# intuitive-robots/beso

Hardware: AMD Instinct MI355X
Metric: denoising-steps/sec (score-GPT fwd) at kitchen obs-dim (higher is better)
Workload: dtype bf16; 1 GPU; BASELINE.json configs[1]: Franka kitchen score-GPT fwd (GCDenoiser.forward), batch=4096 synthetic obs/goal per GPU, 1 NFE per step; obs_dim=30, act_dim=9, window=4, goal_seq_len=2, embed_dim=360, n_layers=6, n_heads=6, batch_per_gpu=4096, parallelism=batch-sharded x1, no collective in the loop, weights=seeded N(0,0.02) recipe (no trained checkpoints shipped)

## Files before the change

### beso_amd/csrc/fused.hip

```cpp
#include <stdlib.h>
#include "fused.h"

#ifndef BESO_OPERAND_F16
#define BESO_OPERAND_F16 0
#endif
#if BESO_OPERAND_F16
#define fused_packed_bytes fused_packed_bytes_f16
#define fused_pack fused_pack_f16
#define fused_level fused_level_f16
#define fused_layer_edges fused_layer_edges_f16
#define fused_layers fused_layers_f16
#define fused_can_loop fused_can_loop_f16
#endif

namespace beso {

typedef __attribute__((ext_vector_type(2))) float f32x2;
typedef __attribute__((ext_vector_type(2))) unsigned int u32x2;

template <int B, int E, typename F>
__device__ __forceinline__ void static_for(F&& f) {
    if constexpr (B < E) {
        f(std::integral_constant<int, B>{});
        static_for<B + 1, E>(f);
// ... 99 lines not shown

constexpr bool kt16(int KS) { return KS == 12 || KS == 8; }

bool shape_has_kernel(const FusedDims& d) {
    if (kt16(d.KS) && d.D > 32 * (d.KS - 1) + 16) return false;
    return (d.RPW == 3 && d.KS == 12) || (d.RPW == 2 && d.KS == 8) || (d.RPW == 4 && d.KS == 16);
}

#if BESO_OPERAND_F16
typedef __attribute__((ext_vector_type(2))) _Float16 f16x2;
typedef __attribute__((ext_vector_type(4))) _Float16 f16x4;
typedef __attribute__((ext_vector_type(8))) _Float16 f16x8;
__device__ __forceinline__ uint16_t f2op(float v) { return __builtin_bit_cast(uint16_t, (_Float16)v); }
__device__ __forceinline__ float op2f(uint16_t h) { return (float)__builtin_bit_cast(_Float16, h); }
#else
__device__ __forceinline__ uint16_t f2op(float v) { return f2bf(v); }
__device__ __forceinline__ float op2f(uint16_t h) { return bf2f(h); }
#endif
__device__ __forceinline__ uint16_t f2op_part(float v, int part) {
    const uint16_t h = f2op(v);
    return part ? f2op(v - op2f(h)) : h;
}

__global__ void pack_mfma_a_kernel(const float* __restrict__ src, int rows, int cols, const float* __restrict__ colscale,
                                   uint16_t* __restrict__ dst, int rt, int kt, int grp, int part) {
    size_t total = (size_t)rt * kt * 512;
    for (size_t i = (size_t)blockIdx.x * blockDim.x + threadIdx.x; i < total; i += (size_t)gridDim.x * blockDim.x) {
        int j = (int)(i & 7), lane = (int)((i >> 3) & 63);
        size_t tile = i >> 9;
        int rin = (int)(tile % grp);
        int kk = (int)((tile / grp) % kt);
        int R = (int)(tile / ((size_t)grp * kt)) * grp + rin;
        int r = 16 * R + (lane & 15);
        int c = 32 * kk + 16 * (j >> 2) + 4 * (lane >> 4) + (j & 3);
        float v = 0.f;
        if (r < rows && c < cols) {
            v = src[(size_t)r * cols + c];
            if (colscale) v *= colscale[c];
        }
        dst[i] = f2op_part(v, part);
    }
}

__global__ void pack_qkv_kernel(const float* __restrict__ wq, const float* __restrict__ wk, const float* __restrict__ wv,
                                const float* __restrict__ gamma, uint16_t* __restrict__ dst, int D, int H, int hd,
                                int kt, int split) {
    size_t total = (size_t)H * 12 * kt * 512;
    for (size_t i = (size_t)blockIdx.x * blockDim.x + threadIdx.x; i < total; i += (size_t)gridDim.x * blockDim.x) {
        int j = (int)(i & 7), lane = (int)((i >> 3) & 63);
        size_t tile = i >> 9;
        int rt12 = (int)(tile % 12);
        int kk = (int)((tile / 24) % kt);
        int h = 2 * (int)(tile / ((size_t)24 * kt)) + (int)((tile / 12) & 1);
        int R4 = rt12 & 3, part = rt12 >> 2;
        int d = 16 * R4 + (lane & 15);
        int c = 32 * kk + 16 * (j >> 2) + 4 * (lane >> 4) + (j & 3);
        float v = 0.f;
        if (d < hd && c < D) {
            const float* w = part == 0 ? wq : (part == 1 ? wk : wv);
            v = w[(size_t)(h * hd + d) * D + c] * gamma[c];
        }
        dst[i] = f2op_part(v, split);
    }
}

__global__ void fold_qkv_bias_kernel(const float* __restrict__ wq, const float* __restrict__ wk,
                                     const float* __restrict__ wv, const float* __restrict__ bq,
                                     const float* __restrict__ bk, const float* __restrict__ bv,
                                     const float* __restrict__ beta, float* __restrict__ out, int D, int H, int hd) {
    const int i = (blockIdx.x * blockDim.x + threadIdx.x) >> 6, lane = threadIdx.x & 63;
    if (i >= H * 3 * kHDP) return;
    int d = i % kHDP, part = (i / kHDP) % 3, h = i / (3 * kHDP);
    float acc = 0.f;
    if (d < hd) {
        const float* w = part == 0 ? wq : (part == 1 ? wk : wv);
        const float* b = part == 0 ? bq : (part == 1 ? bk : bv);
        const int r = h * hd + d;
        for (int c = lane; c < D; c += 64) acc = fmaf(w[(size_t)r * D + c], beta[c], acc);
        acc = wave_sum(acc) + b[r];
    }
    if (lane == 0) out[i] = acc;
}

__global__ void pack_proj_kernel(const float* __restrict__ wp, uint16_t* __restrict__ dst, int D, int H, int hd, int rt,
                                 int part) {
    const int kt = 2 * H;
    size_t total = (size_t)rt * kt * 512;
    for (size_t i = (size_t)blockIdx.x * blockDim.x + threadIdx.x; i < total; i += (size_t)gridDim.x * blockDim.x) {
        int j = (int)(i & 7), lane = (int)((i >> 3) & 63);
        size_t tile = i >> 9;
        int R = (int)(tile % rt), kk = (int)(tile / rt);
        int o = 16 * R + (lane & 15);
        int h = kk >> 1;
        int d = 32 * (kk & 1) + 16 * (j >> 2) + 4 * (lane >> 4) + (j & 3);
        float v = 0.f;
        if (o < D && d < hd) v = wp[(size_t)o * D + h * hd + d];
        dst[i] = f2op_part(v, part);
    }
}

__global__ void transpose_pad_kernel(const float* __restrict__ src, int rows, int cols, float* __restrict__ dst, int rows_p) {
    int i = blockIdx.x * blockDim.x + threadIdx.x;
    if (i >= cols * rows_p) return;
    int c = i / rows_p, f = i % rows_p;
    dst[i] = f < rows ? src[(size_t)f * cols + c] : 0.f;
}

__global__ void pack_head_kernel(const float* __restrict__ W, const float* __restrict__ b, const float* __restrict__ gamma,
                                 const float* __restrict__ beta, float* __restrict__ Wh, float* __restrict__ bh, int act,
                                 int D, int Dp) {
    int i = blockIdx.x * blockDim.x + threadIdx.x;
    if (i < 16 * Dp) {
        int a = i / Dp, f = i % Dp;
        Wh[i] = (a < act && f < D) ? W[(size_t)a * D + f] * gamma[f] : 0.f;
    }
    if (i < 16) {
        float acc = 0.f;
        if (i < act) {
            acc = b[i];
            for (int f = 0; f < D; ++f) acc = fmaf(W[(size_t)i * D + f], beta[f], acc);
        }
        bh[i] = acc;
    }
}

__global__ void fold_bias_kernel(const float* __restrict__ W, const float* __restrict__ b, const float* __restrict__ beta,
                                 float* __restrict__ out, int rows, int cols, int rows_p) {
    const int r = (blockIdx.x * blockDim.x + threadIdx.x) >> 6, lane = threadIdx.x & 63;
    if (r >= rows_p) return;
    float acc = 0.f;
    if (r < rows) {
        for (int c = lane; c < cols; c += 64) acc = fmaf(W[(size_t)r * cols + c], beta[c], acc);
        acc = wave_sum(acc) + b[r];
    }
// ... 47 lines not shown

__device__ __forceinline__ f32x4 mfma_op16(const uint2& a, const uint2& b, const f32x4& c) {
#if BESO_OPERAND_F16
    return __builtin_amdgcn_mfma_f32_16x16x16f16(__builtin_bit_cast(f16x4, a), __builtin_bit_cast(f16x4, b), c, 0, 0, 0);
#else
    return __builtin_amdgcn_mfma_f32_16x16x16bf16_1k(__builtin_bit_cast(s16x4, a), __builtin_bit_cast(s16x4, b), c, 0, 0, 0);
#endif
}

__device__ __forceinline__ f32x4 mfma_op_half(const u32x4& a, const u32x4& b, const f32x4& c) {
    return mfma_op16(make_uint2(a[0], a[1]), make_uint2(b[0], b[1]), c);
}

#ifndef BESO_TRAIN_FWD_ABL
#define BESO_TRAIN_FWD_ABL 0
#endif
__host__ __device__ constexpr bool zero_pad_instance(int RPW, int NT) { return RPW != 2 && NT >= 5; }
__device__ __forceinline__ void mixed_chain_pad() {
    __builtin_amdgcn_sched_barrier(0);
    asm volatile("s_nop 4\n\ts_nop 4");
    __builtin_amdgcn_sched_barrier(0);
}

#ifndef BESO_FUSED_ABLATE
#define BESO_FUSED_ABLATE 0
#endif
#if BESO_FUSED_ABLATE == 1
#define ABL_KS(x) 0
#define ABL_PTR(base, off) (base)
#else
#define ABL_KS(x) (x)
#define ABL_PTR(base, off) ((base).adv(off))
#endif

struct WPtr {
    __amdgpu_buffer_rsrc_t rs;
    uint32_t so;
    uint32_t lo;
    __device__ __forceinline__ u32x4 at(int frag) const {
        return __builtin_amdgcn_raw_buffer_load_b128(rs, lo, so + (uint32_t)frag * 1024u, 0);
    }
    __device__ __forceinline__ WPtr adv(size_t frags) const { return WPtr{rs, so + (uint32_t)frags * 1024u, lo}; }
};
__device__ __forceinline__ WPtr wptr(const u32x4* uniform_base, int lane) {
    return WPtr{__builtin_amdgcn_make_buffer_rsrc((void*)uniform_base, 0, 0x7fffffff, 0x00020000), 0u, (uint32_t)lane * 16u};
}

template <int R>
__device__ __forceinline__ void prefetch_a(u32x4 (&aE)[R], u32x4 (&aO)[R], WPtr a, int a_ks) {
#pragma unroll
    for (int r = 0; r < R; ++r) { aE[r] = a.at(r); aO[r] = a.at(r + ABL_KS(a_ks)); }
}

template <int R, int NT, bool TAIL16 = false, int NTA = NT>
__device__ __forceinline__ void gemm_phase(f32x4 (&acc)[R][NTA], u32x4 (&aE)[R], u32x4 (&aO)[R],
                                           WPtr a, int a_ks, const u32x4* b, int b_ts,
                                           int b_ks, int ksteps) {
    constexpr int H1 = (NT + 1) / 2;
    u32x4 bf[NT];
#pragma unroll
    for (int t = 0; t < NT; ++t) bf[t] = b[t * b_ts];
    for (int kk = 0; kk < ksteps; kk += 2) {
        __builtin_amdgcn_sched_barrier(0);
#pragma unroll
        for (int t = 0; t < H1; ++t)
#pragma unroll
            for (int r = 0; r < R; ++r) acc[r][t] = mfma_op(aE[r], bf[t], acc[r][t]);
        __builtin_amdgcn_sched_barrier(0);
#pragma unroll
        for (int t = 0; t < H1; ++t) if (!(BESO_ABL_MASK & 32)) bf[t] = b[t * b_ts + (kk + 1) * b_ks];
        __builtin_amdgcn_sched_barrier(0);
#pragma unroll
        for (int t = H1; t < NT; ++t)
#pragma unroll
            for (int r = 0; r < R; ++r) acc[r][t] = mfma_op(aE[r], bf[t], acc[r][t]);
        __builtin_amdgcn_sched_barrier(0);
#pragma unroll
        for (int t = H1; t < NT; ++t) if (!(BESO_ABL_MASK & 32)) bf[t] = b[t * b_ts + (kk + 1) * b_ks];
        if (kk + 2 < ksteps) {
#pragma unroll
            for (int r = 0; r < R; ++r) aE[r] = a.at(r + ABL_KS((kk + 2) * a_ks));
        }
        const bool tail = TAIL16 && kk + 2 >= ksteps;
        __builtin_amdgcn_sched_barrier(0);
        if (tail) {
            mixed_chain_pad();
#pragma unroll
            for (int t = 0; t < NT; ++t)
#pragma unroll
                for (int r = 0; r < R; ++r) acc[r][t] = mfma_op_half(aO[r], bf[t], acc[r][t]);
            break;
        }
#pragma unroll
        for (int t = 0; t < H1; ++t)
#pragma unroll
            for (int r = 0; r < R; ++r) acc[r][t] = mfma_op(aO[r], bf[t], acc[r][t]);
        __builtin_amdgcn_sched_barrier(0);
        if (kk + 2 < ksteps && !(BESO_ABL_MASK & 32)) {
#pragma unroll
            for (int t = 0; t < H1; ++t) bf[t] = b[t * b_ts + (kk + 2) * b_ks];
        }
        __builtin_amdgcn_sched_barrier(0);
#pragma unroll
        for (int t = H1; t < NT; ++t)
#pragma unroll
            for (int r = 0; r < R; ++r) acc[r][t] = mfma_op(aO[r], bf[t], acc[r][t]);
        __builtin_amdgcn_sched_barrier(0);
        if (kk + 2 < ksteps && !(BESO_ABL_MASK & 32)) {
#pragma unroll
            for (int t = H1; t < NT; ++t) bf[t] = b[t * b_ts + (kk + 2) * b_ks];
        }
        if (kk + 3 < ksteps) {
#pragma unroll
            for (int r = 0; r < R; ++r) aO[r] = a.at(r + ABL_KS((kk + 3) * a_ks));
        }
    }
}

template <int R, int PFA>
__device__ __forceinline__ void prefetch_ring(u32x4 (&ar)[PFA][R], WPtr a, int a_ks) {
#pragma unroll
    for (int p = 0; p < PFA; ++p)
#pragma unroll
        for (int r = 0; r < R; ++r) ar[p][r] = a.at(r + ABL_KS(p * a_ks));
}

template <int R, int NT, int PFA, bool TAIL16 = false>
__device__ __forceinline__ void gemm_phase_ring(f32x4 (&acc)[R][NT], u32x4 (&ar)[PFA][R],
                                                WPtr a, int a_ks, const u32x4* b, int b_ts,
                                                int b_ks, int ksteps) {
    static_assert(PFA % 2 == 0, "B fragments alternate between two sets");
    u32x4 bb[2][NT];
#pragma unroll
    for (int t = 0; t < NT; ++t) bb[0][t] = b[t * b_ts];
#pragma unroll
    for (int t = 0; t < NT; ++t) bb[1][t] = b[t * b_ts + b_ks];
    for (int k0 = 0; k0 < ksteps; k0 += PFA) {
#pragma unroll
        for (int p = 0; p < PFA; ++p) {
            const int kk = k0 + p;
            __builtin_amdgcn_sched_barrier(0);
            if (TAIL16 && kk + 1 >= ksteps) {
                mixed_chain_pad();
#pragma unroll
                for (int t = 0; t < NT; ++t)
#pragma unroll
                    for (int r = 0; r < R; ++r) acc[r][t] = mfma_op_half(ar[p][r], bb[p & 1][t], acc[r][t]);
            } else {
#pragma unroll
                for (int t = 0; t < NT; ++t)
#pragma unroll
                    for (int r = 0; r < R; ++r) acc[r][t] = mfma_op(ar[p][r], bb[p & 1][t], acc[r][t]);
            }
            __builtin_amdgcn_sched_barrier(0);
            if (BESO_FUSED_ABLATE != 2 && !(BESO_ABL_MASK & 32) && kk + 2 < ksteps) {
#pragma unroll
                for (int t = 0; t < NT; ++t) bb[p & 1][t] = b[t * b_ts + (kk + 2) * b_ks];
            }
            if (BESO_FUSED_ABLATE != 3 && kk + PFA < ksteps) {
// ... 1075 lines not shown
                            gelu_slot<RC, NT, decltype(SG)::value>(h, gc0, gc1, gq, hb);
                        });
                    });
                    __builtin_amdgcn_sched_barrier(0);
                    if (t == H1 - 1 && kk + 1 < kKC && !(BESO_ABL_MASK & 32)) {
#pragma unroll
                        for (int t2 = 0; t2 < H1; ++t2) bf[t2] = b[t2 * kKC * 64 + (kk + 1) * 64];
                    }
                    if (t == NT - 1) {
                        if (kk + 1 < kKC && !(BESO_ABL_MASK & 32)) {
#pragma unroll
                            for (int t2 = H1; t2 < NT; ++t2) bf[t2] = b[t2 * kKC * 64 + (kk + 1) * 64];
                        }
                        if (kk + 2 < kKC) {
#pragma unroll
                            for (int r = 0; r < RPW; ++r) af2[kk & 1][r] = a2.at(r + ABL_KS((kk + 2) * A2KS));
                        }
                    }
                });
            });
        }
        fc2_prefetch(c);
        stamp(st, 21);
        if (!(BESO_ABL_MASK & 2)) __syncthreads();
        stamp(st, 22);
        constexpr bool kLateG = NT <= 4;
        if (fc1_active) { write_hT(hb); if (!kLateG) keep_g(pc(c), hb); }
        if (c + 1 < n_chunks && next_active) { fc1(c + 1, h, a1r); keep_h(pc(c + 1), h); }
        if (kLateG && fc1_active) keep_g(pc(c), hb);
        stamp(st, 23);
        if (!(BESO_ABL_MASK & 2)) __syncthreads();
        stamp(st, 24);
    }
    {
        const int c = n_chunks - 1;
        const int tiles_here = min(kChunkTiles, HT - pc(c) * kChunkTiles);
        gemm_phase<RPW, NT, false, kNTT>(T.acc, af2[0], af2[1], fc2_a(c), A2KS, hT + lane, kKC * 64, 64, ((tiles_here >> 1) + 1) & ~1);
    }
    stamp(st, 25);
    __syncthreads();
}

__device__ __forceinline__ uint2 v_frag(const uint16_t* qkv, int row0, int dt, int n, int g) {
    typedef s16x4 __attribute__((address_space(3))) * lds_s16x4;
    const uint16_t* p = qkv + ((size_t)2 * kQKVRows + row0 + 4 * g + (n >> 2)) * kQKVRow + 16 * dt + 4 * (n & 3);
    return __builtin_bit_cast(uint2, __builtin_amdgcn_ds_read_tr16_b64_v4i16((lds_s16x4)(p)));
}

template <int KS>
__device__ __forceinline__ void attn_prefetch(u32x4 (&qE)[3], u32x4 (&qO)[3], const u32x4* __restrict__ wqkv, int w, int lane) {
    prefetch_a<3>(qE, qO, wptr(wqkv + (size_t)(3 * w) * 64, lane), 24);
}

template <int RPW, int KS, int HG, int NTP = kNTT, int NTQ = kNTT, class AX = AttnPlain>
__device__ __forceinline__ void attn_phase(Tile<RPW>& T, const u32x4* xnT, unsigned char* u,
                                           const u32x4* __restrict__ wqkv, const float* __restrict__ bqkv,
                                           const u32x4* __restrict__ wproj, int H, int hd, int Tn, int n_samples,
                                           int w, int lane, const SlotTabs* tb, u32x4 (&qE)[3], u32x4 (&qO)[3], Stamps& st,
                                           const AX ax = AX{}) {
    asm volatile("" : "+v"(lane));
    uint16_t* qkv = (uint16_t*)u;
    u32x4* yT = (u32x4*)(u + kQKVBytes);
    const int wa = w & 3, hsel = w >> 2;
    const float scale_log2e = 1.4426950408889634f * __builtin_amdgcn_rsqf((float)hd);
    auto qkv_a = [&](int pair) { return ABL_PTR(wptr(wqkv + (size_t)(3 * w) * 64, lane), (size_t)pair * KS * 24); };
    auto proj_a = [&](int h) { return ABL_PTR(wptr(wproj + (size_t)(w * RPW) * 64, lane), (size_t)(2 * h) * (kWaves * RPW)); };
    int ln = lane;
    auto write_qkv = [&](const f32x4 (&qa)[3][NTQ], int vh) {
        const int n = ln & 15, g = ln >> 4;
        int row[NTQ];
#pragma unroll
        for (int t = 0; t < NTQ; ++t) row[t] = tb->row_of_slot[t * 16 + n];
#pragma unroll
        for (int i = 0; i < 3; ++i) {
            const int rt = 3 * wa + i, part = rt >> 2, d0 = (rt & 3) * 16 + 4 * g;
            uint16_t* dst = qkv + (size_t)part * kQKVRows * kQKVRow + d0;
#pragma unroll
            for (int t = 0; t < NTQ; ++t) {
                uint2 pk;
                pk.x = pack_op2(qa[i][t][0], qa[i][t][1]);
                pk.y = pack_op2(qa[i][t][2], qa[i][t][3]);
                *(uint2*)(dst + (size_t)row[t] * kQKVRow) = pk;
                if constexpr (AX::on) {
                    const int grow = ax.rows.row(t * 16 + n);
                    if (grow >= 0 && d0 < HG * hd && !(BESO_TRAIN_FWD_ABL & 4))
                        *(uint2*)(ax.qkv + (size_t)grow * (3 * ax.D) + part * ax.D + vh * (HG * hd) + d0) = pk;
                }
            }
        }
    };
    const int my_tok = tb->slot_of_row[min(w, n_samples - 1) * Tn + min(lane & 15, Tn - 1)];
    auto drop4 = [&](float (&e)[4], int rh, int n, int g) {
        if constexpr (AX::on) {
            if (ax.p > 0.f) {
                const size_t base = drop_idx_attn((size_t)(ax.s0 + w) * ax.H + rh, Tn, n, 4 * g);
#pragma unroll
                for (int r = 0; r < 4; ++r) e[r] *= drop_scale(ax.seed, ax.site, base + r, ax.p, ax.inv_keep);
            }
        }
    };
    auto keep_y = [&](const auto& yb, int vh, int tok, int g) {
        if constexpr (AX::on) {
            const int grow = ax.rows_y.row(tok);
            if (grow >= 0 && !(BESO_TRAIN_FWD_ABL & 4)) {
                uint16_t* dst = ax.y + (size_t)grow * ax.D + vh * (HG * hd) + 4 * g;
#pragma unroll
                for (int dt = 0; dt < 4; ++dt)
                    if (16 * dt + 4 * g < HG * hd) *(uint2*)(dst + 16 * dt) = make_uint2(yb[dt >> 1][2 * (dt & 1)], yb[dt >> 1][2 * (dt & 1) + 1]);
            }
        }
    };
    auto core = [&](int vh) {
    const int n = ln & 15, g = ln >> 4;
    if constexpr (HG > 1) {
        if (w < n_samples && !(BESO_ABL_MASK & 16)) {
            const uint16_t* qb = qkv + ((size_t)0 * kQKVRows + w * Tn + n) * kQKVRow + 8 * g;
            const uint16_t* kb = qkv + ((size_t)1 * kQKVRows + w * Tn + n) * kQKVRow + 8 * g;
            u32x4 qf[2], kf[2];
#pragma unroll
            for (int kk = 0; kk < 2; ++kk) { qf[kk] = *(const u32x4*)(qb + 32 * kk); kf[kk] = *(const u32x4*)(kb + 32 * kk); }
            uint2 va[4];
#pragma unroll
            for (int dt = 0; dt < 4; ++dt) va[dt] = v_frag(qkv, w * Tn, dt, n, g);
            f32x4 y[4];
#pragma unroll
            for (int dt = 0; dt < 4; ++dt) y[dt] = f32x4{0.f, 0.f, 0.f, 0.f};
#pragma unroll
            for (int h = 0; h < HG; ++h) {
                const int lo_d = h * hd, hi_d = lo_d + hd;
                f32x4 sT = {0.f, 0.f, 0.f, 0.f};
#pragma unroll
// ... 60 lines not shown
        float e[4], m = -INFINITY;
#pragma unroll
        for (int r = 0; r < 4; ++r) {
            e[r] = (4 * g + r <= n) ? sT[r] * scale_log2e : -INFINITY;
            m = fmaxf(m, e[r]);
        }
        m = rows_allreduce<true>(m);
        float sum = 0.f;
#pragma unroll
        for (int r = 0; r < 4; ++r) { e[r] = __builtin_amdgcn_exp2f(e[r] - m); sum += e[r]; }
        sum = rows_allreduce<false>(sum);
        const float inv = __builtin_amdgcn_rcpf(sum);
        if constexpr (AX::on) drop4(e, vh, n, g);
        uint2 pb = make_uint2(pack_op2(e[0], e[1]), pack_op2(e[2], e[3]));
        f32x4 y[4];
#pragma unroll
        for (int dt = 0; dt < 4; ++dt) {
            const uint2 va = v_frag(qkv, w * Tn, dt, n, g);
            const f32x4 z = {0.f, 0.f, 0.f, 0.f};
            y[dt] = mfma_op16(va, pb, z);
        }
        if (n < Tn) {
            const int tok = my_tok;
            u32x4 ybk[AX::on ? 2 : 1];
#pragma unroll
            for (int kk = 0; kk < 2; ++kk) {
                u32x4 yb;
                yb[0] = pack_op2(y[2 * kk][0] * inv, y[2 * kk][1] * inv);
                yb[1] = pack_op2(y[2 * kk][2] * inv, y[2 * kk][3] * inv);
                yb[2] = pack_op2(y[2 * kk + 1][0] * inv, y[2 * kk + 1][1] * inv);
                yb[3] = pack_op2(y[2 * kk + 1][2] * inv, y[2 * kk + 1][3] * inv);
                yT[((size_t)(tok >> 4) * 2 + kk) * 64 + (g << 4) + (tok & 15)] = yb;
                if constexpr (AX::on) ybk[kk] = yb;
            }
            if constexpr (AX::on) keep_y(ybk, vh, tok, g);
        }
    }
    }
    };

    for (int pair = 0; pair < H / 2; ++pair) {
        const int hA = 2 * pair, hB = hA + 1;
        asm volatile("" : "+v"(ln));
        const int g = ln >> 4;
        stamp(st, 10);
        u32x4 aE[RPW], aO[RPW];
        f32x4 qa[3][NTQ];
#pragma unroll
        for (int i = 0; i < 3; ++i) {
            const f32x4 bv = *(const f32x4*)(bqkv + ((hA + hsel) * 12 + 3 * wa + i) * 16 + 4 * g);
#pragma unroll
            for (int t = 0; t < NTQ; ++t) qa[i][t] = bv;
        }
        gemm_phase<3, NTQ, kt16(KS)>(qa, qE, qO, qkv_a(pair), 24, xnT + lane, KS * 64, 64, KS);
        prefetch_a<RPW>(aE, aO, proj_a(hA), kWaves * RPW);
        if (hsel == 0) write_qkv(qa, hA);
        stamp(st, 11);
        __syncthreads();
        stamp(st, 12);
        core(hA);
        stamp(st, 16);
        __syncthreads();
        stamp(st, 17);
        gemm_phase<RPW, NTP, false, kNTT>(T.acc, aE, aO, proj_a(hA), kWaves * RPW, yT + lane, 2 * 64, 64, 2);
        prefetch_a<RPW>(aE, aO, proj_a(hB), kWaves * RPW);
        if (hsel == 1) write_qkv(qa, hB);
        if (pair + 1 < H / 2) prefetch_a<3>(qE, qO, qkv_a(pair + 1), 24);
        stamp(st, 13);
        __syncthreads();
        stamp(st, 14);
        core(hB);
        stamp(st, 15);
        __syncthreads();
        stamp(st, 18);
        gemm_phase<RPW, NTP, false, kNTT>(T.acc, aE, aO, proj_a(hB), kWaves * RPW, yT + lane, 2 * 64, 64, 2);
    }
    __syncthreads();
}

template <int RPW, int KS, int NT>
__device__ __forceinline__ void attn_phase_long(Tile<RPW>& T, const u32x4* xnT, unsigned char* u, const u32x4* __restrict__ wqkv,
                                                const float* __restrict__ bqkv, const u32x4* __restrict__ wproj, int H, int hd,
                                                int Tn, int w, int lane, u32x4 (&qE)[3], u32x4 (&qO)[3], Stamps& st) {
    static_assert(NT == 5, "the wave -> query tile table below");
    asm volatile("" : "+v"(lane));
    constexpr int kRows = 16 * NT, kHead = 3 * kRows * kQKVRow;
    constexpr int kYT = 16 * kQKVRow * 2 / 16;
    uint16_t* qkv = (uint16_t*)u;
    const int wa = w & 3, hsel = w >> 2;
    const float scale_log2e = 1.4426950408889634f * __builtin_amdgcn_rsqf((float)hd);
    auto qkv_a = [&](int pair) { return wptr(wqkv + (size_t)(3 * w) * 64, lane).adv((size_t)pair * KS * 24); };
    auto proj_a = [&](int h) { return wptr(wproj + (size_t)(w * RPW) * 64, lane).adv((size_t)(2 * h) * (kWaves * RPW)); };
    int ln = lane;
    auto core = [&](int head, int qt) {
        const int n = ln & 15, g = ln >> 4;
        uint16_t* hq = qkv + (size_t)head * kHead;
        const uint16_t* qb = hq + ((size_t)16 * qt + n) * kQKVRow + 8 * g;
        const u32x4 q0 = *(const u32x4*)qb, q1 = *(const u32x4*)(qb + 32);
        float e[NT][4];
        float m = -INFINITY;
        const int query = 16 * qt + n;
#pragma unroll
        for (int kt = 0; kt < NT; ++kt) {
            if (kt <= qt) {
                const uint16_t* kb = hq + ((size_t)kRows + 16 * kt + n) * kQKVRow + 8 * g;
                f32x4 sT = {0.f, 0.f, 0.f, 0.f};
                sT = mfma_op(*(const u32x4*)kb, q0, sT);
// ... 12 lines not shown
        for (int kt = 0; kt < NT; ++kt) {
            if (kt <= qt) {
#pragma unroll
                for (int r = 0; r < 4; ++r) { e[kt][r] = __builtin_amdgcn_exp2f(e[kt][r] - m); sum += e[kt][r]; }
            }
        }
        sum = rows_allreduce<false>(sum);
        const float inv = __builtin_amdgcn_rcpf(sum);
        f32x4 y[4];
#pragma unroll
        for (int dt = 0; dt < 4; ++dt) y[dt] = f32x4{0.f, 0.f, 0.f, 0.f};
        typedef s16x4 __attribute__((address_space(3))) * lds_s16x4;
#pragma unroll
        for (int kt = 0; kt < NT; ++kt) {
            if (kt <= qt) {
                const uint2 pb = make_uint2(pack_op2(e[kt][0], e[kt][1]), pack_op2(e[kt][2], e[kt][3]));
#pragma unroll
                for (int dt = 0; dt < 4; ++dt) {
                    const uint16_t* pv = hq + ((size_t)2 * kRows + 16 * kt + 4 * g + (n >> 2)) * kQKVRow + 16 * dt + 4 * (n & 3);
                    const uint2 va = __builtin_bit_cast(uint2, __builtin_amdgcn_ds_read_tr16_b64_v4i16((lds_s16x4)(pv)));
                    y[dt] = mfma_op16(va, pb, y[dt]);
                }
            }
        }
        u32x4* yT = (u32x4*)(hq + (size_t)16 * qt * kQKVRow);
#pragma unroll
        for (int kk = 0; kk < 2; ++kk) {
            u32x4 yb;
            yb[0] = pack_op2(y[2 * kk][0] * inv, y[2 * kk][1] * inv);
            yb[1] = pack_op2(y[2 * kk][2] * inv, y[2 * kk][3] * inv);
            yb[2] = pack_op2(y[2 * kk + 1][0] * inv, y[2 * kk + 1][1] * inv);
            yb[3] = pack_op2(y[2 * kk + 1][2] * inv, y[2 * kk + 1][3] * inv);
            yT[kk * 64 + ln] = yb;
        }
    };
#pragma unroll 1
    for (int pair = 0; pair < H / 2; ++pair) {
        const int hA = 2 * pair, hB = hA + 1;
        asm volatile("" : "+v"(ln));
        const int n = ln & 15, g = ln >> 4;
        stamp(st, 10);
        u32x4 aE[RPW], aO[RPW];
        f32x4 qa[3][NT];
#pragma unroll
        for (int i = 0; i < 3; ++i) {
            const f32x4 bv = *(const f32x4*)(bqkv + ((hA + hsel) * 12 + 3 * wa + i) * 16 + 4 * g);
#pragma unroll
            for (int t = 0; t < NT; ++t) qa[i][t] = bv;
        }
        gemm_phase<3, NT, kt16(KS)>(qa, qE, qO, qkv_a(pair), 24, xnT + lane, KS * 64, 64, KS);
        prefetch_a<RPW>(aE, aO, proj_a(hA), kWaves * RPW);
#pragma unroll
        for (int i = 0; i < 3; ++i) {
            const int rt = 3 * wa + i, part = rt >> 2, d0 = (rt & 3) * 16 + 4 * g;
            uint16_t* dst = qkv + (size_t)hsel * kHead + (size_t)part * kRows * kQKVRow + d0;
#pragma unroll
            for (int t = 0; t < NT; ++t)
                *(uint2*)(dst + (size_t)(16 * t + n) * kQKVRow) =
                    make_uint2(pack_op2(qa[i][t][0], qa[i][t][1]), pack_op2(qa[i][t][2], qa[i][t][3]));
        }
        stamp(st, 11);
        __syncthreads();
        stamp(st, 12);
        if (!(BESO_ABL_MASK & 16)) {
            const int head = w & 1, slot = w >> 1;
            core(head, slot == 0 ? 4 : slot == 1 ? 3 : slot == 2 ? 2 : 1);
            if (slot == 2) core(head, 0);
        }
        if (pair + 1 < H / 2) prefetch_a<3>(qE, qO, qkv_a(pair + 1), 24);
        stamp(st, 16);
        __syncthreads();
        stamp(st, 17);
        gemm_phase<RPW, NT, false, kNTT>(T.acc, aE, aO, proj_a(hA), kWaves * RPW, (const u32x4*)qkv + lane, kYT, 64, 2);
        prefetch_a<RPW>(aE, aO, proj_a(hB), kWaves * RPW);
        gemm_phase<RPW, NT, false, kNTT>(T.acc, aE, aO, proj_a(hB), kWaves * RPW, (const u32x4*)(qkv + kHead) + lane, kYT, 64, 2);
        stamp(st, 13);
        __syncthreads();
        stamp(st, 14);
    }
}

__device__ __forceinline__ float gelu_exact(float v) {
    const float ax = fabsf(v) * 0.70710678118654752440f;
    const float t = __builtin_amdgcn_rcpf(fmaf(0.3275911f, ax, 1.0f));
    float p = fmaf(1.061405429f, t, -1.453152027f);
    p = fmaf(p, t, 1.421413741f);
    p = fmaf(p, t, -0.284496736f);
    p = fmaf(p, t, 0.254829592f);
    p *= t;
    const float ex = __builtin_amdgcn_exp2f(ax * ax * -1.4426950408889634f);
    const float r = fmaf(-p, ex, 1.0f);
    const float hv = 0.5f * v;
    return fmaf(fabsf(hv), r, hv);
}

template <int RPW, int KS, int NW, int NT>
__device__ __forceinline__ void mlp_phase_x3(Tile<RPW>& T, const u32x4* xnT, int xn_lo, u32x4* hT, int h_lo,
                                             const u32x4* __restrict__ w1p, const float* __restrict__ b1f,
                                             const u32x4* __restrict__ w2p, int HT, uint32_t x3_delta, int w, int lane) {
    asm volatile("" : "+v"(lane));
    const int n_chunks = (HT + kChunkTiles - 1) / kChunkTiles;
    constexpr int RC = kChunkTiles / NW, KW = RC / 2;
    constexpr int A2KS = NW * RPW;
#pragma unroll 1
    for (int c = 0; c < n_chunks; ++c) {
        asm volatile("" : "+v"(lane));
        const int g = lane >> 4;
// ... 6 lines not shown
#pragma unroll
            for (int t = 0; t < NT; ++t) h[r][t] = bias;
        }
        if (RC * w < tiles_here)
            gemm_x3<RC, NT, 2, kt16(KS)>(h, wptr(w1p + (size_t)(RC * w) * 64, lane).adv((size_t)c * KS * kChunkTiles), kChunkTiles,
                                      x3_delta, xnT + lane, xn_lo, KS * 64, 64, KS);
        u32x4 hh[KW][NT], hl[KW][NT];
#pragma unroll
        for (int j2 = 0; j2 < KW; ++j2)
#pragma unroll
            for (int t = 0; t < NT; ++t)
#pragma unroll
                for (int q = 0; q < 4; ++q) {
                    const f32x4& hv = h[2 * j2 + (q >> 1)][t];
                    const SplitPair p = split_op2(gelu_exact(hv[2 * (q & 1)]), gelu_exact(hv[2 * (q & 1) + 1]));
                    hh[j2][t][q] = p.hi;
                    hl[j2][t][q] = p.lo;
                }
        if (c > 0) __syncthreads();
#pragma unroll
        for (int j2 = 0; j2 < KW; ++j2)
#pragma unroll
            for (int t = 0; t < NT; ++t) {
                hT[((size_t)t * kKC + KW * w + j2) * 64 + lane] = hh[j2][t];
                hT[((size_t)t * kKC + KW * w + j2) * 64 + lane + h_lo] = hl[j2][t];
            }
        __syncthreads();
        gemm_x3<RPW, NT, 2, false, kNTT>(T.acc, wptr(w2p + (size_t)(w * RPW) * 64, lane).adv((size_t)(c * kKC) * A2KS), A2KS, x3_delta,
                                      hT + lane, h_lo, kKC * 64, 64, ((tiles_here >> 1) + 1) & ~1);
    }
    __syncthreads();
}

template <int RPW, int KS, int HG, int NTP, int NTQ>
__device__ __forceinline__ void attn_phase_x3(Tile<RPW>& T, const u32x4* xnT, int xn_lo, unsigned char* u, int qkv_rows,
                                              int y_off, int y_lo, const u32x4* __restrict__ wqkv,
                                              const float* __restrict__ bqkv, const u32x4* __restrict__ wproj, int H, int hd,
                                              int Tn, int n_samples, uint32_t x3_delta, int w, int lane, const SlotTabs* tb) {
    asm volatile("" : "+v"(lane));
    float* qkv = (float*)u;
    u32x4* yT = (u32x4*)(u + y_off);
    const int wa = w & 3, hsel = w >> 2;
    const float scale_log2e = 1.4426950408889634f * __builtin_amdgcn_rsqf((float)hd);
    auto qkv_a = [&](int pair) { return wptr(wqkv + (size_t)(3 * w) * 64, lane).adv((size_t)pair * KS * 24); };
    auto proj_a = [&](int h) { return wptr(wproj + (size_t)(w * RPW) * 64, lane).adv((size_t)(2 * h) * (kWaves * RPW)); };
    int ln = lane;
    auto write_qkv = [&](const f32x4 (&qa)[3][NTQ]) {
        const int n = ln & 15, g = ln >> 4;
#pragma unroll
        for (int t = 0; t < NTQ; ++t) {
            const int row = tb->row_of_slot[t * 16 + n];
#pragma unroll
            for (int i = 0; i < 3; ++i) {
                const int rt = 3 * wa + i, part = rt >> 2, d0 = (rt & 3) * 16 + 4 * g;
                *(f32x4*)(qkv + ((size_t)part * qkv_rows + row) * kQKVRowF + d0) = qa[i][t];
            }
        }
    };
    auto core = [&]() {
        const int n = ln & 15, g = ln >> 4;
        if (w >= n_samples) return;
        const float* qb = qkv + ((size_t)0 * qkv_rows + w * Tn + n) * kQKVRowF + 4 * g;
        const float* kb = qkv + ((size_t)1 * qkv_rows + w * Tn + n) * kQKVRowF + 4 * g;
        const float* vb = qkv + ((size_t)2 * qkv_rows + w * Tn + 4 * g) * kQKVRowF + n;
        f32x4 q4[4], k4[4];
#pragma unroll
        for (int kk = 0; kk < 4; ++kk) { q4[kk] = *(const f32x4*)(qb + 16 * kk); k4[kk] = *(const f32x4*)(kb + 16 * kk); }
        f32x4 y[4];
#pragma unroll
        for (int dt = 0; dt < 4; ++dt) y[dt] = f32x4{0.f, 0.f, 0.f, 0.f};
#pragma unroll
        for (int h = 0; h < HG; ++h) {
            const int lo_d = h * hd, hi_d = lo_d + hd;
            f32x4 sT = {0.f, 0.f, 0.f, 0.f};
#pragma unroll
            for (int kk = 0; kk < 4; ++kk) {
                if (HG > 1 && (16 * kk >= hi_d || 16 * kk + 16 <= lo_d)) continue;
                const int d0 = 16 * kk + 4 * g;
                const bool in = HG == 1 || (d0 >= lo_d && d0 < hi_d);
#pragma unroll
                for (int r = 0; r < 4; ++r)
                    sT = __builtin_amdgcn_mfma_f32_16x16x4f32(k4[kk][r], in ? q4[kk][r] : 0.f, sT, 0, 0, 0);
            }
            float e[4], mx = -INFINITY;
#pragma unroll
            for (int r = 0; r < 4; ++r) {
                e[r] = (4 * g + r <= n) ? sT[r] * scale_log2e : -INFINITY;
                mx = fmaxf(mx, e[r]);
            }
            mx = rows_allreduce<true>(mx);
            float sum = 0.f;
#pragma unroll
            for (int r = 0; r < 4; ++r) { e[r] = __builtin_amdgcn_exp2f(e[r] - mx); sum += e[r]; }
            sum = rows_allreduce<false>(sum);
            const float inv = 1.0f / sum;
#pragma unroll
            for (int dt = 0; dt < 4; ++dt) {
                if (HG > 1 && (16 * dt >= hi_d || 16 * dt + 16 <= lo_d)) continue;
                f32x4 yh = {0.f, 0.f, 0.f, 0.f};
#pragma unroll
                for (int r = 0; r < 4; ++r)
                    yh = __builtin_amdgcn_mfma_f32_16x16x4f32(vb[(size_t)r * kQKVRowF + 16 * dt], e[r], yh, 0, 0, 0);
                const int d0 = 16 * dt + 4 * g;
                const bool mine = HG == 1 || (d0 >= lo_d && d0 < hi_d);
#pragma unroll
                for (int r = 0; r < 4; ++r) y[dt][r] = mine ? yh[r] * inv : y[dt][r];
            }
// ... 345 lines not shown
            for (int t = 0; t < kNTT; ++t) qa[i][t] = bv;
        }
        u32x4 aE[RPW], aO[RPW];
        const WPtr wq = wptr((const u32x4*)(lw_next + ti.o_wqkv + (size_t)part * ti.part_bytes) + (size_t)(w * RPW) * 64, lane);
        prefetch_a<RPW>(aE, aO, wq, kWaves * RPW);
        gemm_phase<RPW, kNTT, kt16(KS)>(qa, aE, aO, wq, kWaves * RPW, xnT + lane, KS * 64, 64, KS);
#pragma unroll
        for (int i = 0; i < RPW; ++i) {
            const int f0 = 16 * (w * RPW + i) + 4 * gg;
            if (f0 < d.D) {
#pragma unroll
                for (int t = 0; t < kNTT; ++t) {
                    const int tok = m0 + 16 * t + nn;
                    if (tok < M)
                        *(uint2*)(a.qkvn + (size_t)tok * ldq + (size_t)part * d.D + f0) =
                            make_uint2(pack_op2(qa[i][t][0], qa[i][t][1]), pack_op2(qa[i][t][2], qa[i][t][3]));
                }
            }
        }
    }
}

struct TrainPackSeg { const float* src; uint32_t dst; int rows, cols, rt, kt, grp, first_block, tr; };
constexpr int kTrainPackSegs = 96;
struct TrainPackTable { TrainPackSeg seg[kTrainPackSegs]; int n, blocks; };
struct TrainPackBuilder {
    TrainPackTable t;
    TrainPackBuilder() { t.n = 0; t.blocks = 0; }
    void seg(const float* src, uint32_t dst, int rows, int cols, int rt, int kt, int grp, int tr, size_t elems) {
        t.seg[t.n++] = TrainPackSeg{src, dst, rows, cols, rt, kt, grp, t.blocks, tr};
        t.blocks += rt == 0 ? 1 : (int)((elems + 256 * 16 - 1) / (256 * 16));
    }
    void mat(const float* src, uint32_t dst, int rows, int cols, int rt, int kt, int grp, int tr = 0) {
        seg(src, dst, rows, cols, rt, kt, grp, tr, (size_t)rt * kt * 512);
    }
    void vec(const float* src, uint32_t dst, int n, int n_pad) { seg(src, dst, n, n_pad, 0, 0, 0, 0, 0); }
};
__global__ void train_pack_kernel(TrainPackTable t, char* __restrict__ img) {
    __shared__ int which;
    if (threadIdx.x == 0) {
        int lo = 0, hi = t.n - 1;
        while (lo < hi) { const int mid = (lo + hi + 1) >> 1; if (t.seg[mid].first_block <= (int)blockIdx.x) lo = mid; else hi = mid - 1; }
        which = lo;
    }
    __syncthreads();
    const TrainPackSeg& g = t.seg[which];
    const int nb = (which + 1 < t.n ? t.seg[which + 1].first_block : t.blocks) - g.first_block;
    const size_t start = (size_t)(blockIdx.x - g.first_block) * blockDim.x + threadIdx.x, stride = (size_t)nb * blockDim.x;
    if (g.rt == 0) {
        float* dst = (float*)(img + g.dst);
        if (g.tr == 4) {
            for (size_t i = start; i < (size_t)g.cols; i += stride) {
                const int hv = (int)(i >> 6), dd = (int)(i & 63);
                dst[((size_t)hv * 3 + g.grp) * kHDP + dd] = dd < g.rows ? g.src[(size_t)hv * g.rows + dd] : 0.f;
            }
            return;
        }
        for (size_t i = start; i < (size_t)g.cols; i += stride) dst[i] = i < (size_t)g.rows ? g.src[i] : 0.f;
        return;
    }
    uint16_t* dst = (uint16_t*)(img + g.dst);
    const uint32_t total8 = (uint32_t)g.rt * (uint32_t)g.kt * 64u * (g.tr == 2 ? 4u : 1u);
    const bool vec_ok = ((uintptr_t)g.src & 15) == 0;
    auto put8 = [&](uint32_t i8, uint32_t dst8, bool row_ok, const float* row, int c0, int ncols, size_t cstride) {
        float v[8];
        if (row_ok && cstride == 1 && vec_ok && c0 + 20 <= ncols && (ncols & 3) == 0) {
            const f32x4 lo = *(const f32x4*)(row + c0), hi = *(const f32x4*)(row + c0 + 16);
#pragma unroll
            for (int j = 0; j < 4; ++j) { v[j] = lo[j]; v[4 + j] = hi[j]; }
        } else {
#pragma unroll
            for (int j = 0; j < 8; ++j) {
                const int c = c0 + 16 * (j >> 2) + (j & 3);
                v[j] = (row_ok && c < ncols) ? row[(size_t)c * cstride] : 0.f;
            }
        }
        u32x4 o;
#pragma unroll
        for (int j = 0; j < 4; ++j) o[j] = (uint32_t)f2bf(v[2 * j]) | ((uint32_t)f2bf(v[2 * j + 1]) << 16);
        *(u32x4*)(dst + (size_t)dst8 * 8) = o;
    };
    const uint32_t start8 = (uint32_t)start, stride8 = (uint32_t)stride;
    if (g.tr == 2) {
        for (uint32_t i8 = start8; i8 < total8; i8 += stride8) {
            const uint32_t lane = i8 & 63, tile = i8 >> 6;
            const uint32_t R4 = tile & 3, kk = (tile >> 2) % (uint32_t)g.kt, h = tile / (4u * (uint32_t)g.kt);
            const int dd = 16 * (int)R4 + (int)(lane & 15), c0 = 32 * (int)kk + 4 * (int)(lane >> 4);
            const uint32_t dtile = ((h >> 1) * (uint32_t)g.kt + kk) * 24 + (h & 1) * 12 + (uint32_t)g.grp * 4 + R4;
            put8(i8, dtile * 64 + lane, dd < g.rows, g.src + ((size_t)h * g.rows + (dd < g.rows ? dd : 0)) * g.cols, c0, g.cols, 1);
        }
        return;
    }
    if (g.tr == 3) {
        for (uint32_t i8 = start8; i8 < total8; i8 += stride8) {
            const uint32_t lane = i8 & 63, tile = i8 >> 6;
            const uint32_t R = tile % (uint32_t)g.rt, kk = tile / (uint32_t)g.rt;
            const int o = 16 * (int)R + (int)(lane & 15), h = (int)(kk >> 1), d0 = 32 * (int)(kk & 1) + 4 * (int)(lane >> 4);
            float v[8];
#pragma unroll
            for (int j = 0; j < 8; ++j) {
                const int dd = d0 + 16 * (j >> 2) + (j & 3);
                v[j] = (o < g.rows && dd < g.cols) ? g.src[(size_t)o * g.rows + h * g.cols + dd] : 0.f;
            }
            u32x4 ov;
#pragma unroll
            for (int j = 0; j < 4; ++j) ov[j] = (uint32_t)f2bf(v[2 * j]) | ((uint32_t)f2bf(v[2 * j + 1]) << 16);
            *(u32x4*)(dst + (size_t)i8 * 8) = ov;
        }
        return;
    }
    for (uint32_t i8 = start8; i8 < total8; i8 += stride8) {
        const uint32_t lane = i8 & 63, tile = i8 >> 6;
        const uint32_t rin = tile % (uint32_t)g.grp, kk = (tile / (uint32_t)g.grp) % (uint32_t)g.kt;
        const uint32_t R = tile / ((uint32_t)g.grp * (uint32_t)g.kt) * (uint32_t)g.grp + rin;
        const int r = 16 * (int)R + (int)(lane & 15), c0 = 32 * (int)kk + 4 * (int)(lane >> 4);
        const bool rv = r < g.rows;
        if (g.tr) put8(i8, i8, rv, g.src + (rv ? r : 0), c0, g.cols, (size_t)g.rows);
        else put8(i8, i8, rv, g.src + (size_t)(rv ? r : 0) * g.cols, c0, g.cols, 1);
    }
}

template <int NT, int KS>
struct LdsMapLinX3 {
    static constexpr int a_bytes = NT * KS * 1024, a_lo = a_bytes / 16;
    static constexpr int hT = 2 * a_bytes, h_bytes = NT * kKCc * 1024, h_lo = h_bytes / 16;
    static constexpr int red = hT + 2 * h_bytes, total = red + kRedTok * kMT * 4;
};
template <int RPW, int KS, int NT>
__global__ __launch_bounds__(512, 2) void lin_block_x3_kernel(float* __restrict__ x, const char* __restrict__ lw,
                                                              const char* __restrict__ lw_next, FusedDims d, int M,
                                                              const float* __restrict__ y, int ld_y, float* __restrict__ qkv) {
    Stamps st{nullptr, 0, 0};
    extern __shared__ __attribute__((aligned(16))) unsigned char lds[];
    using L = LdsMapLinX3<NT, KS>;
    static_assert(L::total <= 160 * 1024, "LDS of the split-bf16 block kernel");
    int lane = threadIdx.x & 63;
    const int w = __builtin_amdgcn_readfirstlane(threadIdx.x >> 6);
    const int m0 = blockIdx.x * 16 * NT;
    u32x4* aT = (u32x4*)lds;
    float* red = (float*)(lds + L::red);
    Tile<RPW> T;
// ... 144 lines not shown
#endif
    };
    if constexpr (PX) {
        auto layer_x3 = [&](const char* lw, auto NTPc) {
            constexpr int NTP = decltype(NTPc)::value;
            u32x4* xnT = (u32x4*)(lds + L.xnT);
            layernorm_to_lds<RPW, KS, kWaves, true, NTA, 1>(T, xnT, (float*)(lds + L.red), d.D, w, lane,
                                                            (const float*)(lw + d.o_bproj), st, X.xn_lo);
            attn_phase_x3<RPW, KS, HG, NTP, NTA>(T, xnT, X.xn_lo, lds + L.u, X.qkv_rows, X.yT, X.y_lo,
                                                 (const u32x4*)(lw + d.o_wqkv), (const float*)(lw + d.o_bqkv),
                                                 (const u32x4*)(lw + d.o_wproj), d.Hv, d.hd, Tn, n_samples, d.x3_delta, w, lane, tb);
            layernorm_to_lds<RPW, KS, kWaves, true, NTP, 1>(T, xnT, (float*)(lds + L.red), d.D, w, lane,
                                                            (const float*)(lw + d.o_b2), st, X.xn_lo);
            mlp_phase_x3<RPW, KS, kWaves, NTP>(T, xnT, X.xn_lo, (u32x4*)(lds + L.u), X.h_lo, (const u32x4*)lw,
                                               (const float*)(lw + d.o_b1), (const u32x4*)(lw + d.o_w2), d.HT, d.x3_delta, w, lane);
        };
#pragma unroll 1
        for (int l = l0; l < l_loop_end; ++l) layer_x3(layer_weights(l), std::integral_constant<int, NTA>{});
        if (peel) layer_x3(layer_weights(l1 - 1), std::integral_constant<int, NTLa>{});
    } else {
    for (int l = l0; l < l_loop_end; ++l) {
        const char* lw = layer_weights(l);
        stamp(st, 2);
        u32x4 qE[3], qO[3];
        attn_prefetch<KS>(qE, qO, (const u32x4*)(lw + d.o_wqkv), w, lane);
        layernorm_to_lds<RPW, KS, kWaves, true, NTA>(T, (u32x4*)(lds + L.xnT), (float*)(lds + L.red), d.D, w, lane,
                                          (const float*)(lw + d.o_bproj), st, 0, LnPlain{}, n_valid);
        stamp(st, 7);
        if constexpr (CORE == 1)
            attn_phase_long<RPW, KS, NTA>(T, (const u32x4*)(lds + L.xnT), lds + L.u, (const u32x4*)(lw + d.o_wqkv),
                                          (const float*)(lw + d.o_bqkv), (const u32x4*)(lw + d.o_wproj), d.Hv, d.hd, Tn, w, lane,
                                          qE, qO, st);
        else
        attn_phase<RPW, KS, HG, NTA, NTA>(T, (const u32x4*)(lds + L.xnT), lds + L.u, (const u32x4*)(lw + d.o_wqkv),
                                (const float*)(lw + d.o_bqkv), (const u32x4*)(lw + d.o_wproj), d.Hv, d.hd, Tn, n_samples, w,
                                lane, tb, qE, qO, st);
        stamp(st, 3);
        u32x4 a1r[PF1][kChunkTiles / kWaves];
        mlp_prefetch<KS, kWaves, PF1>(a1r, (const u32x4*)lw, w, lane);
        layernorm_to_lds<RPW, KS, kWaves, true, NTA>(T, (u32x4*)(lds + L.xnT), (float*)(lds + L.red), d.D, w, lane,
                                          (const float*)(lw + d.o_b2), st, 0, LnPlain{}, n_valid);
        stamp(st, 6);
        mlp_phase<RPW, KS, kWaves, NTA, PF1>(T, (const u32x4*)(lds + L.xnT), (u32x4*)(lds + L.u), (const u32x4*)lw,
                                   (const float*)(lw + d.o_b1), (const u32x4*)(lw + d.o_w2), d.HT, d.KS2p, w, lane, a1r, st, MlpPlain{}, n_valid);
    }
    if (peel) {
        const char* lw = layer_weights(l1 - 1);
        stamp(st, 2);
        u32x4 qE[3], qO[3];
        attn_prefetch<KS>(qE, qO, (const u32x4*)(lw + d.o_wqkv), w, lane);
        layernorm_to_lds<RPW, KS, kWaves, true, NTA>(T, (u32x4*)(lds + L.xnT), (float*)(lds + L.red), d.D, w, lane,
                                          (const float*)(lw + d.o_bproj), st, 0, LnPlain{}, n_valid);
        stamp(st, 7);
        attn_phase<RPW, KS, HG, NTLa, NTA>(T, (const u32x4*)(lds + L.xnT), lds + L.u, (const u32x4*)(lw + d.o_wqkv),
                                     (const float*)(lw + d.o_bqkv), (const u32x4*)(lw + d.o_wproj), d.Hv, d.hd, Tn, n_samples, w,
                                     lane, tb, qE, qO, st);
        stamp(st, 3);
        u32x4 a1r[PF1][kChunkTiles / kWaves];
        mlp_prefetch<KS, kWaves, PF1>(a1r, (const u32x4*)lw, w, lane);
        layernorm_to_lds<RPW, KS, kWaves, true, NTLa>(T, (u32x4*)(lds + L.xnT), (float*)(lds + L.red), d.D, w, lane,
                                                     (const float*)(lw + d.o_b2), st);
        stamp(st, 6);
        mlp_phase<RPW, KS, kWaves, NTLa, PF1>(T, (const u32x4*)(lds + L.xnT), (u32x4*)(lds + L.u), (const u32x4*)lw,
                                        (const float*)(lw + d.o_b1), (const u32x4*)(lw + d.o_w2), d.HT, d.KS2p, w, lane, a1r, st);
    }
    }
    stamp(st, 4);
    if constexpr (LOOP) {
        const StepRec rec = S.rec[ev];
        ls.mode = rec.mode; ls.c0 = rec.c0; ls.c1 = rec.c1; ls.c2 = rec.c2; ls.c3 = X3.c3[ev]; ls.ev = rec.mode >> kStepShift;
        ls.last = ev + 1 == n_evals;
    }
    {
        if constexpr (CORE == 1) head_tile<RPW, NTA, LOOP != 0>(T, e, d, gw, (float*)(lds + L.red), (float*)(lds + L.u), s0p, n_samples, Tn, w, lane, tb, xs, ls, st,
                                                     two_pass ? pass : -1, (float*)(lds + L.cfgc));
        else if (peel && NTLa < kNTT) head_tile<RPW, NTLa, LOOP != 0>(T, e, d, gw, (float*)(lds + L.red), (float*)(lds + L.u), s0, n_samples, Tn, w, lane, tb, xs, ls, st);
        else head_tile<RPW, kNTT, LOOP != 0>(T, e, d, gw, (float*)(lds + L.red), (float*)(lds + L.u), s0, n_samples, Tn, w, lane, tb, xs, ls, st);
    }
    stamp(st, 5);
    if (CORE == 1 && pass + 1 < n_pass) __syncthreads();
    }
    if (LOOP && ev + 1 < n_evals) __syncthreads();
    }
    stamp(st, 101);
}

struct TrainImgW { uint32_t o_ln1w, o_ln1b, o_ln2w, o_ln2b, layer_bytes; };
static TrainImgW train_img_whole(const FusedDims& d) {
    TrainImgW t;
    const uint32_t vec = (uint32_t)round_up_sz((size_t)d.RPW * kWaves * 16 * sizeof(float), 256);
    t.o_ln1w = d.layer_bytes; t.o_ln1b = t.o_ln1w + vec; t.o_ln2w = t.o_ln1b + vec; t.o_ln2b = t.o_ln2w + vec;
    t.layer_bytes = t.o_ln2b + vec;
    return t;
}

template <int RPW, int KS, int HG, int NTL, int SPW, int NTA, int RD = 0>
__global__ __launch_bounds__(512, 2) void train_fwd_kernel(const char* __restrict__ img, FusedDims d, TrainImgW ti,
                                                           int n_samples_total, int Tn, TrainWholeBufs a) {
    Stamps st{nullptr, 0, 0};
    extern __shared__ __attribute__((aligned(16))) unsigned char lds[];
    constexpr LdsMap L = lds_map(KS);
    constexpr int NTLa = NTL < NTA ? NTL : NTA;
    constexpr int PF1 = NTA < kNTT ? kFc1PFLat : kFc1PF;
    const int lane = threadIdx.x & 63;
    const int w = __builtin_amdgcn_readfirstlane(threadIdx.x >> 6);
    const int s0 = blockIdx.x * SPW;
    const int n_samples = min(SPW, n_samples_total - s0);
// ... 1156 lines not shown
```

Baseline: 1213 denoise-steps/s (one step = GCDenoiser.forward over B=4096 samples per GPU).

## Interleave QKV row tiles per wave and skip unused query rows in last layer

Repacks the fused QKV weight and bias so each wave's three row tiles are Q, K and V for the same 16 head dims, rather than a strided slice of the 12 tiles. With that layout the first accumulator row of every wave is always Q, so the GEMM can skip MFMAs for Q row-tiles beyond NTQROW. In the peeled last layer only the rows the attention output actually needs get Q computed and written. This cuts tensor-core work in the final layer's QKV projection. The cost is a layout change that every pack path, bias fold and write_qkv indexing site must follow consistently.

```diff
diff --git a/beso_amd/csrc/fused.hip b/beso_amd/csrc/fused.hip
--- a/beso_amd/csrc/fused.hip
+++ b/beso_amd/csrc/fused.hip
@@ -175,7 +175,7 @@
         int rt12 = (int)(tile % 12);
         int kk = (int)((tile / 24) % kt);
         int h = 2 * (int)(tile / ((size_t)24 * kt)) + (int)((tile / 12) & 1);
-        int R4 = rt12 & 3, part = rt12 >> 2;
+        int R4 = rt12 / 3, part = rt12 % 3;
         int d = 16 * R4 + (lane & 15);
         int c = 32 * kk + 16 * (j >> 2) + 4 * (lane >> 4) + (j & 3);
         float v = 0.f;
@@ -202,7 +202,7 @@
         for (int c = lane; c < D; c += 64) acc = fmaf(w[(size_t)r * D + c], beta[c], acc);
         acc = wave_sum(acc) + b[r];
     }
-    if (lane == 0) out[i] = acc;
+    if (lane == 0) out[((h * 4 + (d >> 4)) * 3 + part) * 16 + (d & 15)] = acc;
 }
 
 __global__ void pack_proj_kernel(const float* __restrict__ wp, uint16_t* __restrict__ dst, int D, int H, int hd, int rt,
@@ -356,7 +356,7 @@
     for (int r = 0; r < R; ++r) { aE[r] = a.at(r); aO[r] = a.at(r + ABL_KS(a_ks)); }
 }
 
-template <int R, int NT, bool TAIL16 = false, int NTA = NT>
+template <int R, int NT, bool TAIL16 = false, int NTA = NT, int NT0 = NT>
 __device__ __forceinline__ void gemm_phase(f32x4 (&acc)[R][NTA], u32x4 (&aE)[R], u32x4 (&aO)[R],
                                            WPtr a, int a_ks, const u32x4* b, int b_ts,
                                            int b_ks, int ksteps) {
@@ -369,7 +369,7 @@
 #pragma unroll
         for (int t = 0; t < H1; ++t)
 #pragma unroll
-            for (int r = 0; r < R; ++r) acc[r][t] = mfma_op(aE[r], bf[t], acc[r][t]);
+            for (int r = 0; r < R; ++r) if (r > 0 || t < NT0) acc[r][t] = mfma_op(aE[r], bf[t], acc[r][t]);
         __builtin_amdgcn_sched_barrier(0);
 #pragma unroll
         for (int t = 0; t < H1; ++t) if (!(BESO_ABL_MASK & 32)) bf[t] = b[t * b_ts + (kk + 1) * b_ks];
@@ -377,7 +377,7 @@
 #pragma unroll
         for (int t = H1; t < NT; ++t)
 #pragma unroll
-            for (int r = 0; r < R; ++r) acc[r][t] = mfma_op(aE[r], bf[t], acc[r][t]);
+            for (int r = 0; r < R; ++r) if (r > 0 || t < NT0) acc[r][t] = mfma_op(aE[r], bf[t], acc[r][t]);
         __builtin_amdgcn_sched_barrier(0);
 #pragma unroll
         for (int t = H1; t < NT; ++t) if (!(BESO_ABL_MASK & 32)) bf[t] = b[t * b_ts + (kk + 1) * b_ks];
@@ -392,13 +392,13 @@
 #pragma unroll
             for (int t = 0; t < NT; ++t)
 #pragma unroll
-                for (int r = 0; r < R; ++r) acc[r][t] = mfma_op_half(aO[r], bf[t], acc[r][t]);
+                for (int r = 0; r < R; ++r) if (r > 0 || t < NT0) acc[r][t] = mfma_op_half(aO[r], bf[t], acc[r][t]);
             break;
         }
 #pragma unroll
         for (int t = 0; t < H1; ++t)
 #pragma unroll
-            for (int r = 0; r < R; ++r) acc[r][t] = mfma_op(aO[r], bf[t], acc[r][t]);
+            for (int r = 0; r < R; ++r) if (r > 0 || t < NT0) acc[r][t] = mfma_op(aO[r], bf[t], acc[r][t]);
         __builtin_amdgcn_sched_barrier(0);
         if (kk + 2 < ksteps && !(BESO_ABL_MASK & 32)) {
 #pragma unroll
@@ -408,7 +408,7 @@
 #pragma unroll
         for (int t = H1; t < NT; ++t)
 #pragma unroll
-            for (int r = 0; r < R; ++r) acc[r][t] = mfma_op(aO[r], bf[t], acc[r][t]);
+            for (int r = 0; r < R; ++r) if (r > 0 || t < NT0) acc[r][t] = mfma_op(aO[r], bf[t], acc[r][t]);
         __builtin_amdgcn_sched_barrier(0);
         if (kk + 2 < ksteps && !(BESO_ABL_MASK & 32)) {
 #pragma unroll
@@ -1590,12 +1590,13 @@
     prefetch_a<3>(qE, qO, wptr(wqkv + (size_t)(3 * w) * 64, lane), 24);
 }
 
-template <int RPW, int KS, int HG, int NTP = kNTT, int NTQ = kNTT, class AX = AttnPlain>
+template <int RPW, int KS, int HG, int NTP = kNTT, int NTQ = kNTT, class AX = AttnPlain, int NTQROW = NTQ>
 __device__ __forceinline__ void attn_phase(Tile<RPW>& T, const u32x4* xnT, unsigned char* u,
                                            const u32x4* __restrict__ wqkv, const float* __restrict__ bqkv,
                                            const u32x4* __restrict__ wproj, int H, int hd, int Tn, int n_samples,
                                            int w, int lane, const SlotTabs* tb, u32x4 (&qE)[3], u32x4 (&qO)[3], Stamps& st,
                                            const AX ax = AX{}) {
+    static_assert(!AX::on || NTQROW == NTQ, "the training forward keeps every q row for the backward pass");
     asm volatile("" : "+v"(lane));
     uint16_t* qkv = (uint16_t*)u;
     u32x4* yT = (u32x4*)(u + kQKVBytes);
@@ -1611,10 +1612,10 @@
         for (int t = 0; t < NTQ; ++t) row[t] = tb->row_of_slot[t * 16 + n];
 #pragma unroll
         for (int i = 0; i < 3; ++i) {
-            const int rt = 3 * wa + i, part = rt >> 2, d0 = (rt & 3) * 16 + 4 * g;
+            const int part = i, d0 = wa * 16 + 4 * g;
             uint16_t* dst = qkv + (size_t)part * kQKVRows * kQKVRow + d0;
 #pragma unroll
-            for (int t = 0; t < NTQ; ++t) {
+            for (int t = 0; t < (i == 0 ? NTQROW : NTQ); ++t) {
                 uint2 pk;
                 pk.x = pack_op2(qa[i][t][0], qa[i][t][1]);
                 pk.y = pack_op2(qa[i][t][2], qa[i][t][3]);
@@ -1781,7 +1782,7 @@
 #pragma unroll
             for (int t = 0; t < NTQ; ++t) qa[i][t] = bv;
         }
-        gemm_phase<3, NTQ, kt16(KS)>(qa, qE, qO, qkv_a(pair), 24, xnT + lane, KS * 64, 64, KS);
+        gemm_phase<3, NTQ, kt16(KS), NTQ, NTQROW>(qa, qE, qO, qkv_a(pair), 24, xnT + lane, KS * 64, 64, KS);
         prefetch_a<RPW>(aE, aO, proj_a(hA), kWaves * RPW);
         if (hsel == 0) write_qkv(qa, hA);
         stamp(st, 11);
@@ -1900,7 +1901,7 @@
         prefetch_a<RPW>(aE, aO, proj_a(hA), kWaves * RPW);
 #pragma unroll
         for (int i = 0; i < 3; ++i) {
-            const int rt = 3 * wa + i, part = rt >> 2, d0 = (rt & 3) * 16 + 4 * g;
+            const int part = i, d0 = wa * 16 + 4 * g;
             uint16_t* dst = qkv + (size_t)hsel * kHead + (size_t)part * kRows * kQKVRow + d0;
 #pragma unroll
             for (int t = 0; t < NT; ++t)
@@ -2013,7 +2014,7 @@
             const int row = tb->row_of_slot[t * 16 + n];
 #pragma unroll
             for (int i = 0; i < 3; ++i) {
-                const int rt = 3 * wa + i, part = rt >> 2, d0 = (rt & 3) * 16 + 4 * g;
+                const int part = i, d0 = wa * 16 + 4 * g;
                 *(f32x4*)(qkv + ((size_t)part * qkv_rows + row) * kQKVRowF + d0) = qa[i][t];
             }
         }
@@ -2465,7 +2466,7 @@
         if (g.tr == 4) {
             for (size_t i = start; i < (size_t)g.cols; i += stride) {
                 const int hv = (int)(i >> 6), dd = (int)(i & 63);
-                dst[((size_t)hv * 3 + g.grp) * kHDP + dd] = dd < g.rows ? g.src[(size_t)hv * g.rows + dd] : 0.f;
+                dst[(((size_t)hv * 4 + (dd >> 4)) * 3 + g.grp) * 16 + (dd & 15)] = dd < g.rows ? g.src[(size_t)hv * g.rows + dd] : 0.f;
             }
             return;
         }
@@ -2499,7 +2500,7 @@
             const uint32_t lane = i8 & 63, tile = i8 >> 6;
             const uint32_t R4 = tile & 3, kk = (tile >> 2) % (uint32_t)g.kt, h = tile / (4u * (uint32_t)g.kt);
             const int dd = 16 * (int)R4 + (int)(lane & 15), c0 = 32 * (int)kk + 4 * (int)(lane >> 4);
-            const uint32_t dtile = ((h >> 1) * (uint32_t)g.kt + kk) * 24 + (h & 1) * 12 + (uint32_t)g.grp * 4 + R4;
+            const uint32_t dtile = ((h >> 1) * (uint32_t)g.kt + kk) * 24 + (h & 1) * 12 + R4 * 3 + (uint32_t)g.grp;
             put8(i8, dtile * 64 + lane, dd < g.rows, g.src + ((size_t)h * g.rows + (dd < g.rows ? dd : 0)) * g.cols, c0, g.cols, 1);
         }
         return;
@@ -2750,7 +2751,7 @@
         layernorm_to_lds<RPW, KS, kWaves, true, NTA>(T, (u32x4*)(lds + L.xnT), (float*)(lds + L.red), d.D, w, lane,
                                           (const float*)(lw + d.o_bproj), st, 0, LnPlain{}, n_valid);
         stamp(st, 7);
-        attn_phase<RPW, KS, HG, NTLa, NTA>(T, (const u32x4*)(lds + L.xnT), lds + L.u, (const u32x4*)(lw + d.o_wqkv),
+        attn_phase<RPW, KS, HG, NTLa, NTA, AttnPlain, NTLa>(T, (const u32x4*)(lds + L.xnT), lds + L.u, (const u32x4*)(lw + d.o_wqkv),
                                      (const float*)(lw + d.o_bqkv), (const u32x4*)(lw + d.o_wproj), d.Hv, d.hd, Tn, n_samples, w,
                                      lane, tb, qE, qO, st);
         stamp(st, 3);
```

Result: no change. 1221 denoise-steps/s (one step = GCDenoiser.forward over B=4096 samples per GPU), median of 6 (+0.7%).
